# E-J408/admm-net

Measured on AMD Instinct MI355X. Metric: signals/sec (K-layer ADMM-Net forward), higher is better.
Workload: dtype f32; 1 GPU; cfg3: ADMMNet K=16 grid 16x16 (D=256, n=257) batch 65536/GPU + spectrum on 1024 atoms; batch_per_gpu=65536, global_batch=65536, K=16, D=256, n=257, natoms=1024, batch_mean_scope=global, chunk=8192, weights=torch.manual_seed(0) default init, glayer=matrix function, checked per matrix; eigensolver on the rejected matrices

## Files before the change

__graft_entry__.py:

```python
import os
import subprocess
import sys

ROOT = os.path.dirname(os.path.abspath(__file__))
if ROOT not in sys.path:
    sys.path.insert(0, ROOT)


def build() -> None:
    from admm_net_amd import build as b
    lib = b.build_extension()
    assert os.path.exists(lib)
    for name in ("eigh_model", "dc_model", "arrow_model"):
        so = os.path.join(ROOT, "tests", "host_model", "lib%s.so" % name)
        subprocess.check_call(["g++", "-O2", "-shared", "-fPIC", "-I", os.path.join(ROOT, "admm_net_amd", "csrc"),
                               os.path.join(ROOT, "tests", "host_model", name + ".cpp"), "-o", so])
    import admm_net_amd
    from admm_net_amd import _lib
    _lib.load()


def smoke() -> None:
    import numpy as np
    import torch
    import admm_net_amd as A
    from admm_net_amd import synth
    from oracle import admm_net_ref as R
    assert torch.cuda.is_available(), "smoke() needs the GPU"
    dev = torch.device("cuda:0")
    Nb, Nd, K, B = 4, 4, 3, 5
    sd = R.make_weights(Nb, Nd, K, seed=1, head=True, perturb=0.3)
    m = A.ADMMNet(M=Nb, N=Nd, num_layers=K).eval()
    m.load_state_dict(sd)
    y, b, s, _ = synth.make_batch(B, Nb, Nd, seed=2)
    ty, tb, ts = torch.from_numpy(y), torch.from_numpy(b), torch.from_numpy(s)
    tau, f, conf, phi = m(ty.to(dev), tb.to(dev), ts.to(dev))
    torch.cuda.synchronize()
    ref = R.forward(sd, ty, tb, ts, Nb, Nd, K, head=True)
    err = float(np.abs(phi.cpu().numpy() - ref[3].numpy()).max() / np.abs(ref[3].numpy()).max())
    herr = max(float((a.cpu() - r).abs().max()) for a, r in zip((tau, f, conf), ref[:3]))
    assert err < 1e-4 and herr < 5e-5, (err, herr)
    st = m.last_status
    print(f"smoke ok: phi rel err {err:.2e}, head abs err {herr:.2e}; G-layer routes {st}")


if __name__ == "__main__":
    build()
    if "--smoke" in sys.argv:
        smoke()
```

admm_net_amd/csrc/arrow.hip:

```cpp
#include <cstdio>
#include <cstdlib>

#include "common.h"

#include "arrow_core.h"
#include "rebuild_lds.h"

namespace admmnet {

constexpr int AR_THREADS = 256;

struct ArShared {
    int k, nrot, conf;
    int mx[2];
    float znorm;
};

__host__ __device__ inline size_t ar_np(int D) { return (size_t)((D + 1 + 3) & ~3); }
__host__ __device__ inline size_t ar_lds_bytes(const BrGeom &g) {
    const size_t NP = ar_np(g.D);
    return sizeof(float) * (g.vt_floats() + g.small_floats() + 12 * NP) + sizeof(int) * 5 * NP + sizeof(DcRot) * NP;
}

template <bool BIG>
__global__ __launch_bounds__(AR_THREADS, 1) void arrow_rebuild_kernel(
    int D, const float *__restrict__ lw, const float2 *__restrict__ phi, const float *__restrict__ h,
    float2 *__restrict__ G, float *__restrict__ rn, float *__restrict__ w_out, int32_t *__restrict__ status,
    unsigned long long *__restrict__ ptime, int lower_only, float *VTg, float *__restrict__ w0g) {
    extern __shared__ __attribute__((aligned(16))) char smem[];
    __shared__ ArShared sh;
    long long t_prev = ptime ? clock64() : 0;
    auto mark = [&](int id) {
        if (ptime && threadIdx.x == 0) {
            const long long t_now = clock64();
            atomicAdd(&ptime[id], (unsigned long long)(t_now - t_prev));
            t_prev = t_now;
        }
    };
    const BrGeom g(D);
    const int n = g.n;
    const int Dp = BIG ? D : g.Dp, VP = BIG ? 2 * D : g.VP;
    const int NP = (int)ar_np(D);
    const int tid = threadIdx.x;
    const int64_t b = blockIdx.x;
    const float alpha = lw[S_CORNER_G];
    float *VTl = BIG ? VTg + b * ((int64_t)n * 2 * D) : reinterpret_cast<float *>(smem);
    float *fs = reinterpret_cast<float *>(smem) + (BIG ? 0 : g.vt_floats());
    float *w0f = fs + ((n + 4) & ~3);
    float *z0s = w0f + ((n + 4) & ~3);
    float *rowb = z0s + ((n + 4) & ~3);
    float *redb = rowb + 2 * Dp;
    float *hraw = redb + 8;
    float *zraw = hraw + NP;
    float *phr = zraw + NP;
    float *phim = phr + NP;
    float *ds = phim + NP;
    float *zs = ds + NP;
    float *dl = zs + NP;
    float *zl = dl + NP;
    float *tau = zl + NP;
    float *zh = tau + NP;
    float *vals = zh + NP;
    float *x0 = vals + NP;
    float *lamd = zs;
    int *perm = reinterpret_cast<int *>(x0 + NP);
    int *src = perm + NP;
    int *org = src + NP;
    int *rnk = org + NP;
    int *kidx = rnk + NP;
    DcRot *rot = reinterpret_cast<DcRot *>(kidx + NP);

    if (tid == 0) {
        sh.mx[0] = __float_as_int(fabsf(alpha));
        sh.mx[1] = 0;
    }
    int bad = 0;
    for (int i = tid; i < D; i += AR_THREADS) {
        const float2 z = phi[b * D + i];
        const float a = sqrtf(z.x * z.x + z.y * z.y);
        const float ia = a > 0.f ? 1.0f / a : 0.f;
        hraw[i] = h[b * D + i];
        bad |= !(isfinite(a) && isfinite(hraw[i]));
        zraw[i] = a;
        phr[i] = a > 0.f ? z.x * ia : 1.f;
        phim[i] = a > 0.f ? z.y * ia : 0.f;
    }
    if (__syncthreads_or(bad)) {
        if (tid == 0 && status) atomicAdd(status, 1);
        return;
    }
    for (int i = tid; i < D; i += AR_THREADS) {
        const float v = hraw[i];
        int r = 0;
#pragma unroll 8
        for (int q = 0; q < D; ++q) {
            const float u = hraw[q];
            r += (u < v) || (u == v && q < i);
        }
        perm[r] = i;
        ds[r] = v;
        zs[r] = zraw[i];
        atomicMax(&sh.mx[0], __float_as_int(fabsf(v)));
        atomicMax(&sh.mx[1], __float_as_int(zraw[i]));
    }
    __syncthreads();
    {
        const float dmax = __int_as_float(sh.mx[0]), zmax = __int_as_float(sh.mx[1]);
        int trig = 0;
        for (int p = tid; p < D; p += AR_THREADS) trig |= deflate_triggers(p, 1.0f, dmax, zmax, ds, zs) ? 1 : 0;
        if (__syncthreads_or(trig)) {
            const float tol = 8.0f * kEps32 * fmaxf(dmax, zmax);
            float *dde = reinterpret_cast<float *>(kidx);
            defl_par_flags(tid, AR_THREADS, D, 1.0f, tol, ds, zs, org, rnk, tau, zh);
            if (tid == 0) sh.conf = 0;
            __syncthreads();
            defl_par_walk(tid, AR_THREADS, D, tol, ds, zs, org, rnk, tau, zh, vals, x0, dde, &sh.conf);
            __syncthreads();
            if (sh.conf) {
                if (tid == 0) {
                    int k = 0, nr = 0;
                    deflate_scan_tol(D, 1.0f, dmax, zmax, ds, zs, dl, zl, src, rot, k, nr);
                    sh.k = k;
                    sh.nrot = nr;
                }
            } else {
                defl_par_emit(tid, AR_THREADS, D, ds, org, rnk, tau, zh, vals, x0, dde, dl, zl, src, rot, &sh.k, &sh.nrot);
            }
        } else {
            for (int p = tid; p < D; p += AR_THREADS) {
                dl[p] = ds[p];
                zl[p] = zs[p];
                src[p] = p;
            }
            if (tid == 0) {
                sh.k = D;
                sh.nrot = 0;
            }
        }
    }
    __syncthreads();
    mark(0);
    const int k = sh.k, nrot = sh.nrot;
    for (int p = k + tid; p < D; p += AR_THREADS) vals[p + 1] = dl[p];
    for (int p = tid; p < D; p += AR_THREADS) kidx[src[p]] = (p < k) ? p : -(p + 1) - 1;
    if (tid < 64) {
        float s = 0.f;
        for (int i = tid; i < k; i += 64) s = fmaf(zl[i], zl[i], s);
        s = wave_sum(s);
        if (tid == 0) sh.znorm = sqrtf(s);
    }
    __syncthreads();
    if (k == 0) {
        if (tid == 0) vals[0] = alpha;
    } else {
        const float znorm = sh.znorm;
        auto put = [&](int jr, int o, float t) {
            org[jr] = o;
            tau[jr] = t;
            lamd[jr] = dl[o];
            vals[jr] = dl[o] + t;
        };
        const int first = (k + 1 <= AR_THREADS / 2 + 1) ? min(k + 1, AR_THREADS / 2) : min(k + 1, AR_THREADS);
        if (first <= AR_THREADS / 2) {
            const int jr = tid >> 1, sub = tid & 1;
            if (jr < first) {
                int o;
                float t;
                arrow_root(k, jr, alpha, znorm, dl, zl, o, t, nullptr, sub, 2, [](float x) {
                    return x + __builtin_bit_cast(float, __builtin_amdgcn_update_dpp(0, __builtin_bit_cast(int, x), 0xB1,
                                                                                       0xF, 0xF, false));
                });
                if (sub == 0) put(jr, o, t);
            }
        } else if (tid < first) {
            int o;
            float t;
            arrow_root(k, tid, alpha, znorm, dl, zl, o, t);
            put(tid, o, t);
        }
        if (tid < 64) {
            for (int jr = first; jr <= k; ++jr) {
                int o;
                float t;
                arrow_root(k, jr, alpha, znorm, dl, zl, o, t, nullptr, tid, 64, [](float x) { return wave_sum(x); });
                if (tid == 0) put(jr, o, t);
            }
        }
    }
    __syncthreads();
    for (int p = tid; p < n; p += AR_THREADS) bad |= !isfinite(vals[p]);
    mark(1);
    {
        const int G = (2 * k <= AR_THREADS) ? 2 : 1;
        const int sub = (G == 2) ? (tid & 1) : 0;
        auto redm = [G](float x) {
            const float y = __builtin_bit_cast(
                float, __builtin_amdgcn_update_dpp(0, __builtin_bit_cast(int, x), 0xB1, 0xF, 0xF, false));
            return G == 2 ? x * y : x;
        };
        for (int i = (G == 2) ? (tid >> 1) : tid; i < k; i += AR_THREADS / G) {
            const float v = arrow_zhat(k, i, dl, lamd, tau, sub, G, redm);
            if (sub == 0) zh[i] = v;
        }
    }
    for (int s = tid; s < n; s += AR_THREADS) {
        const float v = vals[s];
        int r = 0;
#pragma unroll 8
        for (int q = 0; q < n; ++q) {
            const float u = vals[q];
            r += (u < v) || (u == v && q < s);
        }
        rnk[s] = r;
    }
    __syncthreads();
    {
        const LayerLayout L{D};
        const float thr = lw[S_THR];
        const float *vn = lw + L.off_vn();
        for (int s = tid; s < n; s += AR_THREADS) {
            float xa = 0.f;
            if (s <= k) {
                float nrm = 1.f;
                if (k > 0) {
                    const float dorg = lamd[s], ts = tau[s];
#pragma unroll 4
                    for (int i = 0; i < k; ++i) {
                        const float v = fdiv_fast(zh[i], (dorg - dl[i]) + ts);
                        nrm = fmaf(v, v, nrm);
                    }
                }
                xa = 1.0f / sqrtf(nrm);
            }
            x0[s] = xa;
            const int c = rnk[s];
            const float lam = vals[s];
            const float f = br_eig_map(lam, thr, vn);
            fs[c] = f;
            w0f[c] = xa * f;
            z0s[c] = xa;
            if (w_out) w_out[b * n + c] = lam;
            if (BIG) w0g[b * n + c] = xa;
        }
        if (tid == 0) {
            fs[n] = 0.f;
            w0f[n] = 0.f;
            z0s[n] = 0.f;
        }
    }
    __syncthreads();
    mark(2);
    int *ipos = reinterpret_cast<int *>(hraw);
    for (int p = tid; p < D; p += AR_THREADS) ipos[perm[p]] = p;
    __syncthreads();
    const int nparts = (AR_THREADS / Dp > 0) ? AR_THREADS / Dp : 1;
    const int sper = (n + nparts - 1) / nparts;
    for (int it = tid; it < Dp * nparts; it += AR_THREADS) {
        const int i = it % Dp, part = it / Dp;
        const int s0 = part * sper, s1 = min(n, s0 + sper);
        float *colr = VTl + i, *coli = VTl + Dp + i;
        if (i >= D) {
            for (int c = s0; c < s1; ++c) {
                colr[c * VP] = 0.f;
                coli[c * VP] = 0.f;
            }
            continue;
        }
        const int kd = kidx[ipos[i]];
        if (kd >= 0) {
            const float zi = zh[kd], di = dl[kd];
#pragma unroll 4
            for (int s = s0; s < min(s1, k + 1); ++s) {
                const float v = fdiv_fast(zi, (lamd[s] - di) + tau[s]) * x0[s];
                colr[rnk[s] * VP] = v;
            }
            for (int s = max(s0, k + 1); s < s1; ++s) colr[rnk[s] * VP] = 0.f;
        } else {
            const int slot = -kd - 1;
#pragma unroll 4
            for (int s = s0; s < s1; ++s) colr[rnk[s] * VP] = (s == slot) ? 1.f : 0.f;
        }
    }
    __syncthreads();
    for (int c = tid; c < n; c += AR_THREADS) {
        float *row = VTl + c * VP;
        for (int r = nrot - 1; r >= 0; --r) {
            const DcRot rr = rot[r];
            const int ia = perm[rr.pa], ib = perm[rr.pb];
            const float a = row[ia], bb = row[ib];
            row[ia] = rr.c * a - rr.s * bb;
            row[ib] = rr.s * a + rr.c * bb;
        }
    }
    __syncthreads();
    for (int it = tid; it < Dp * nparts; it += AR_THREADS) {
        const int i = it % Dp, part = it / Dp;
        if (i >= D) continue;
        float *colr = VTl + i, *coli = VTl + Dp + i;
        const float pr = phr[i], pi = phim[i];
#pragma unroll 8
        for (int c = part * sper; c < min(n, (part + 1) * sper); ++c) {
            const float x = colr[c * VP];
            colr[c * VP] = x * pr;
            coli[c * VP] = x * pi;
        }
    }
    __syncthreads();
    mark(3);
    if (__syncthreads_or(bad) && tid == 0 && status) atomicAdd(status, 1);
    if constexpr (BIG) return;
    else rebuild_from_lds(g, b, lw, VTl, fs, w0f, z0s, rowb, redb, phi, h, G, rn, [&](int id) { mark(id); }, lower_only);
}

bool arrow_rebuild_supported(int D) { return D >= 1 && D <= 256; }

int launch_arrow_rebuild(int D, int64_t nb, const float *lw, const float2 *phi, const float *h, float2 *G, float *rn,
                         float *w_out, int32_t *status, const Ws &ws, hipStream_t st, bool lower_only) {
    if (nb <= 0) return ADMMNET_OK;
    if (!arrow_rebuild_supported(D)) {
        set_error("arrow_rebuild: D=%d unsupported", D);
        return ADMMNET_E_ARG;
    }
    const BrGeom g(D);
    if (D > 128) {
        {
            ProfScope _prof(KC_REBUILD, st);
            const size_t lds = ar_lds_bytes(g) - sizeof(float) * g.vt_floats();
            ADMM_HIP(hipFuncSetAttribute(reinterpret_cast<const void *>(arrow_rebuild_kernel<true>),
                                         hipFuncAttributeMaxDynamicSharedMemorySize, (int)lds));
            hipLaunchKernelGGL(arrow_rebuild_kernel<true>, dim3((unsigned)nb), dim3(AR_THREADS), lds, st, D, lw, phi, h,
                               G, rn, ws.w, status, (unsigned long long *)nullptr, lower_only ? 1 : 0, ws.VT, ws.w0);
            ADMM_HIP(hipGetLastError());
        }
        return launch_rebuild(D, nb, lw, phi, h, G, rn, w_out, ws, st, lower_only, D);
    }
    ProfScope _prof(KC_REBUILD, st);
    const size_t lds = ar_lds_bytes(g);
    ADMM_HIP(hipFuncSetAttribute(reinterpret_cast<const void *>(arrow_rebuild_kernel<false>),
                                 hipFuncAttributeMaxDynamicSharedMemorySize, (int)lds));
    static const bool timing = getenv("ADMMNET_AR_TIMING") != nullptr;
    unsigned long long *ptime = nullptr;
    if (timing) {
        ADMM_HIP(hipMalloc(&ptime, 16 * sizeof(unsigned long long)));
        ADMM_HIP(hipMemsetAsync(ptime, 0, 16 * sizeof(unsigned long long), st));
    }
    hipLaunchKernelGGL(arrow_rebuild_kernel<false>, dim3((unsigned)nb), dim3(AR_THREADS), lds, st, D, lw, phi, h, G, rn,
                       w_out, status, ptime, lower_only ? 1 : 0, (float *)nullptr, (float *)nullptr);
    ADMM_HIP(hipGetLastError());
    if (timing) {
        unsigned long long hb[16];
        ADMM_HIP(hipMemcpyAsync(hb, ptime, sizeof(hb), hipMemcpyDeviceToHost, st));
        ADMM_HIP(hipStreamSynchronize(st));
        ADMM_HIP(hipFree(ptime));
        static const char *nm[6] = {"sort+deflate", "roots", "zhat+rank+norm", "vectors", "G tiles", "arrow+norm"};
        fprintf(stderr, "[arrow_rebuild timing] D=%d nb=%lld  mean cycles per workgroup:\n", D, (long long)nb);
        for (int i = 0; i < 6; ++i) fprintf(stderr, "   %-14s %10.0f\n", nm[i], (double)hb[i] / (double)nb);
    }
    return ADMMNET_OK;
}

}
```

admm_net_amd/csrc/arrow_core.h:

```cpp
#pragma once
#include "dc_core.h"

namespace admmnet {

struct ArrowEval {
    float w, dpsi, dphi, err;
};

struct ArrowNoReduce {
    HD float operator()(float x) const { return x; }
};

template <class DA, class ZA, class Red = ArrowNoReduce>
HD ArrowEval arrow_eval(int k, int jsplit, float c0, float dorg, float t, DA d, ZA z, int sub = 0, int G = 1,
                        Red red = Red()) {
    float sum = 0.f, asum = 0.f, dall = 0.f, dps = 0.f;
#pragma unroll 4
    for (int i = sub; i < k; i += G) {
        const float del = (d(i) - dorg) - t;
        const float r = fdiv_fast(1.0f, del);
        const float zi = z(i);
        const float term = zi * zi * r;
        const float dterm = term * r;
        sum += term;
        asum += fabsf(term);
        dall += dterm;
        dps += (i <= jsplit) ? dterm : 0.f;
    }
    sum = red(sum);
    asum = red(asum);
    dall = red(dall);
    dps = red(dps);
    ArrowEval e;
    e.w = (c0 + t) + sum;
    e.dpsi = dps;
    e.dphi = dall - dps;
    e.err = 8.0f * asum + fabsf(c0) + 2.0f * fabsf(t) + fabsf(t) * dall;
    return e;
}

template <class DA, class ZA, class Red = ArrowNoReduce>
HD void arrow_root_upper(int k, int j, float alpha, float znorm, DA d, ZA z, int &org_out, float &tau_out,
                         int *nit = nullptr, int sub = 0, int G = 1, Red red = Red()) {
    if (nit) *nit = 0;
    const bool top = (j == k);
    int org, plo, phi_;
    float lo, hi, t;
    ArrowEval e;
    if (top) {
        org = k - 1;
        plo = (k >= 2) ? k - 2 : k - 1;
        phi_ = k - 1;
        const float bq = d(k - 1) - alpha;
        const float disc = sqrtf(bq * bq + 4.0f * znorm * znorm);
        hi = (bq > 0.f) ? 2.0f * znorm * znorm / (bq + disc) : 0.5f * (disc - bq);
        lo = 0.f;
        if (k == 1) {
            org_out = org;
            tau_out = hi;
            return;
        }
        hi = hi * (1.0f + 8.0f * kEps32) + 1e-30f;
        t = hi;
        e = arrow_eval(k, plo, d(org) - alpha, d(org), t, d, z, sub, G, red);
        if (e.w <= 0.f) {
            org_out = org;
            tau_out = hi;
            return;
        }
    } else {
        plo = j - 1;
        phi_ = j;
        const float half = 0.5f * (d(j) - d(j - 1));
        e = arrow_eval(k, plo, d(j - 1) - alpha, d(j - 1), half, d, z, sub, G, red);
        if (e.w >= 0.f) {
            org = j - 1;
            lo = 0.f;
            hi = half;
            t = half;
        } else {
            org = j;
            lo = -half;
            hi = 0.f;
            t = -half;
        }
    }
    const float dorg = d(org), c0 = dorg - alpha;
    const float plo_off = d(plo) - dorg, phi_off = d(phi_) - dorg;
    for (int it = 0; it < 60; ++it) {
        if (nit) *nit = it + 1;
        if (fabsf(e.w) <= kEps32 * e.err) break;
        if (e.w < 0.f) lo = t; else hi = t;
        const float d1 = plo_off - t, d2 = phi_off - t;
        const float dw = e.dpsi + e.dphi + 1.0f;
        float c = e.w - d1 * e.dpsi - d2 * e.dphi;
        const float aa = (d1 + d2) * e.w - d1 * d2 * (e.dpsi + e.dphi);
        const float bb = d1 * d2 * e.w;
        float eta;
        if (top) {
            const float zk = z(k - 1), z2 = zk * zk;
            const float psi = e.w - (c0 + t) + fdiv_fast(z2, t);
            const float B = 1.0f + e.dpsi, A = c0 + psi - e.dpsi * t;
            const float disc = sqrtf(A * A + 4.0f * B * z2);
            const float tq = (A > 0.f) ? fdiv_fast(2.0f * z2, A + disc) : fdiv_fast(disc - A, 2.0f * B);
            eta = tq - t;
            (void)c; (void)aa; (void)bb;
        } else {
            if (c == 0.f) {
                eta = (aa != 0.f) ? fdiv_fast(bb, aa) : 0.f;
            } else {
                const float disc = sqrtf(fabsf(aa * aa - 4.0f * bb * c));
                eta = (aa <= 0.f) ? fdiv_fast(aa - disc, 2.0f * c) : fdiv_fast(2.0f * bb, aa + disc);
            }
        }
        if (!(e.w * eta < 0.f)) eta = -fdiv_fast(e.w, dw);
        float tn = t + eta;
        if (!(tn > lo && tn < hi)) tn = 0.5f * (lo + hi);
        if (tn == t || tn == lo || tn == hi) break;
        t = tn;
        e = arrow_eval(k, plo, c0, dorg, t, d, z, sub, G, red);
    }
    if (t == 0.f) t = (lo == 0.f) ? 0.5f * hi : 0.5f * lo;
    if (t == 0.f) t = (lo == 0.f) ? 1e-30f : -1e-30f;
    org_out = org;
    tau_out = t;
}

template <class FA, class Red = ArrowNoReduce>
HD void arrow_root(int k, int j, float alpha, float znorm, FA d, FA z, int &org_out, float &tau_out,
                   int *nit = nullptr, int sub = 0, int G = 1, Red red = Red()) {
    const bool refl = (j == 0);
    const float sg = refl ? -1.0f : 1.0f;
    const int km1 = k - 1;
    int orgr;
    float taur;
    arrow_root_upper(k, refl ? k : j, sg * alpha, znorm, [&](int i) { return sg * d[refl ? km1 - i : i]; },
                     [&](int i) { return z[refl ? km1 - i : i]; }, orgr, taur, nit, sub, G, red);
    org_out = refl ? km1 - orgr : orgr;
    tau_out = sg * taur;
}

template <class FA>
HD float arrow_delta(FA d, FA lamd, FA tau, int i, int j) {
    return (d[i] - lamd[j]) - tau[j];
}

template <class FA, class Red = ArrowNoReduce>
HD float arrow_zhat(int k, int i, FA d, FA lamd, FA tau, int sub = 0, int G = 1, Red red = Red()) {
    const float di = d[i];
    float w = (sub == 0) ? ((di - lamd[i]) - tau[i]) * -((di - lamd[i + 1]) - tau[i + 1])
                         : 1.0f;
#pragma unroll 4
    for (int j = sub; j < k; j += G) {
        const int jr = (j < i) ? j : j + 1;
        const float q = fdiv_fast((di - lamd[jr]) - tau[jr], di - d[j]);
        w *= (j == i) ? 1.0f : q;
    }
    return sqrtf(fabsf(red(w)));
}

}
```

Measured before the change: 87740 signals/s.

## Fuse arrow eigenvector generation and G rebuild into one MFMA kernel for large D

For D>128 the arrow rebuild now runs a fused path by default. Instead of writing the full eigenvector matrix VT to global scratch and running a separate rebuild pass, it generates eigenvector rows in 16-row LDS slabs (double-buffered), undoes the deflation rotations, and accumulates X·diag(f)·X^T with fp32 MFMA 32x32x2 directly. The phase, the arrow row and the residual norm are applied in the epilogue. This removes the global VT round trip and the separate G build, and allows two workgroups per CU, at the cost of register pressure from nine 16-wide accumulators and added complexity in the rotation replay.

After: 92470 signals/s, median of 6. +5.4%, better.

```diff
diff --git a/__graft_entry__.py b/__graft_entry__.py
--- a/__graft_entry__.py
+++ b/__graft_entry__.py
@@ -11,7 +11,7 @@
     from admm_net_amd import build as b
     lib = b.build_extension()
     assert os.path.exists(lib)
-    for name in ("eigh_model", "dc_model", "arrow_model"):
+    for name in ("eigh_model", "dc_model", "arrow_model", "arrow_fused_model"):
         so = os.path.join(ROOT, "tests", "host_model", "lib%s.so" % name)
         subprocess.check_call(["g++", "-O2", "-shared", "-fPIC", "-I", os.path.join(ROOT, "admm_net_amd", "csrc"),
                                os.path.join(ROOT, "tests", "host_model", name + ".cpp"), "-o", so])
diff --git a/admm_net_amd/csrc/arrow.hip b/admm_net_amd/csrc/arrow.hip
--- a/admm_net_amd/csrc/arrow.hip
+++ b/admm_net_amd/csrc/arrow.hip
@@ -9,6 +9,10 @@
 namespace admmnet {
 
 constexpr int AR_THREADS = 256;
+enum ArMode { AR_LDS = 0, AR_GLOBAL = 1, AR_FUSED = 2 };
+constexpr int AF_KS = 16;
+constexpr int AF_W = kMaxD;
+static_assert(AR_THREADS == AF_W, "the fused tail gives every thread one column of X");
 
 struct ArShared {
     int k, nrot, conf;
@@ -22,11 +26,186 @@
     return sizeof(float) * (g.vt_floats() + g.small_floats() + 12 * NP) + sizeof(int) * 5 * NP + sizeof(DcRot) * NP;
 }
 
-template <bool BIG>
-__global__ __launch_bounds__(AR_THREADS, 1) void arrow_rebuild_kernel(
+using f32x16 = __attribute__((ext_vector_type(16))) float;
+
+template <class Mark>
+__device__ __forceinline__ void arrow_fused_tail(int D, int nrot, int64_t b, const float *__restrict__ lw, float *slab,
+                                                 const float *fs, const float *w0f, const float *z0s, const float *lamc,
+                                                 const float *tauc, const float *phr, const float *phim, const float *zh,
+                                                 const float *dl, const int *kidx, int *ipos, const int *perm,
+                                                 const int *rnk, const DcRot *rot, float *redb,
+                                                 const float2 *__restrict__ phi, const float *__restrict__ h,
+                                                 float2 *__restrict__ G, float *__restrict__ rn, int lower_only, Mark mark) {
+    const int n = D + 1, NT = (D + 31) >> 5;
+    const int tid = threadIdx.x, lane = tid & 63;
+    const int wave = __builtin_amdgcn_readfirstlane(tid >> 6);
+    const int r32 = lane & 31, kh = lane >> 5;
+    const int Ihi = 7 - wave, Ilo = wave;
+    for (int p = tid; p < D; p += AR_THREADS) ipos[perm[p]] = p;
+    __syncthreads();
+    float zi = 0.f, di = 0.f;
+    int cdef = -1;
+    bool surv = false;
+    if (tid < D) {
+        const int kd = kidx[ipos[tid]];
+        if (kd >= 0) {
+            surv = true;
+            zi = zh[kd];
+            di = dl[kd];
+        } else {
+            cdef = rnk[-kd - 1];
+        }
+    }
+    auto gen = [&](int sl, int buf) {
+        float *dst = slab + buf * (AF_KS * AF_W) + tid;
+        const int c0 = sl * AF_KS;
+#pragma unroll
+        for (int r = 0; r < AF_KS; ++r) {
+            const int c = c0 + r, cc = min(c, n - 1);
+            const float v = surv ? arrow_vec_entry(zi, di, lamc[cc], tauc[cc], z0s[cc]) : (c == cdef ? 1.f : 0.f);
+            dst[r * AF_W] = (c < n) ? v : 0.f;
+        }
+    };
+    auto unrotate = [&](int sl, int buf) {
+        const int r = tid >> 4;
+        if ((tid & 15) == 0 && sl * AF_KS + r < n) {
+            float *row = slab + (buf * AF_KS + r) * AF_W;
+            for (int q = nrot - 1; q >= 0; --q) {
+                const DcRot rr = rot[q];
+                const int ia = perm[rr.pa], ib = perm[rr.pb];
+                const float a = row[ia], bb = row[ib];
+                row[ia] = rr.c * a - rr.s * bb;
+                row[ib] = rr.s * a + rr.c * bb;
+            }
+        }
+    };
+    const bool hi5 = 5 <= Ihi, hi6 = 6 <= Ihi, hi7 = 7 <= Ihi;
+    const int J5 = hi5 ? 5 : 3, J6 = hi6 ? 6 : 2, J7 = hi7 ? 7 : 1;
+    const bool en_hi = Ihi < NT, en_lo = Ilo < NT;
+    const bool en5 = hi5 ? en_hi : en_lo, en6 = hi6 ? en_hi : en_lo, en7 = hi7 ? en_hi : en_lo;
+    f32x16 acc[9];
+#pragma unroll
+    for (int q = 0; q < 9; ++q) acc[q] = f32x16{0};
+    float arow = 0.f;
+    const int nslab = (n + AF_KS - 1) / AF_KS;
+    gen(0, 0);
+    __syncthreads();
+    if (nrot > 0) {
+        unrotate(0, 0);
+        __syncthreads();
+    }
+    mark(3);
+    auto consume = [&](int sl) {
+        const int c0 = sl * AF_KS;
+        const float *sb = slab + (sl & 1) * (AF_KS * AF_W);
+#pragma unroll
+        for (int r = 0; r < AF_KS; ++r) arow = fmaf(w0f[min(c0 + r, n)], sb[r * AF_W + tid], arow);
+        struct Step { float x0, x1, x2, x3, x4, x5, x6, x7, ahi, alo; };
+        auto load = [&](int kk) {
+            const float fc = fs[min(c0 + kk + kh, n)];
+            const float *row = sb + (kk + kh) * AF_W + r32;
+            return Step{row[0], row[32], row[64], row[96], row[128], row[32 * J5], row[32 * J6], row[32 * J7],
+                        row[32 * Ihi] * fc, row[32 * Ilo] * fc};
+        };
+        Step cur = load(0);
+#pragma unroll
+        for (int kk = 0; kk < AF_KS; kk += 2) {
+            Step nxt = cur;
+            if (kk + 2 < AF_KS) nxt = load(kk + 2);
+            __builtin_amdgcn_sched_barrier(0);
+            if (c0 + kk < n) {
+                const float a5 = hi5 ? cur.ahi : cur.alo, a6 = hi6 ? cur.ahi : cur.alo, a7 = hi7 ? cur.ahi : cur.alo;
+                if (en_hi) {
+                    acc[0] = __builtin_amdgcn_mfma_f32_32x32x2f32(cur.ahi, cur.x0, acc[0], 0, 0, 0);
+                    acc[1] = __builtin_amdgcn_mfma_f32_32x32x2f32(cur.ahi, cur.x1, acc[1], 0, 0, 0);
+                    acc[2] = __builtin_amdgcn_mfma_f32_32x32x2f32(cur.ahi, cur.x2, acc[2], 0, 0, 0);
+                    acc[3] = __builtin_amdgcn_mfma_f32_32x32x2f32(cur.ahi, cur.x3, acc[3], 0, 0, 0);
+                    acc[4] = __builtin_amdgcn_mfma_f32_32x32x2f32(cur.ahi, cur.x4, acc[4], 0, 0, 0);
+                }
+                if (en5) acc[5] = __builtin_amdgcn_mfma_f32_32x32x2f32(a5, cur.x5, acc[5], 0, 0, 0);
+                if (en6) acc[6] = __builtin_amdgcn_mfma_f32_32x32x2f32(a6, cur.x6, acc[6], 0, 0, 0);
+                if (en7) acc[7] = __builtin_amdgcn_mfma_f32_32x32x2f32(a7, cur.x7, acc[7], 0, 0, 0);
+                if (en_lo) acc[8] = __builtin_amdgcn_mfma_f32_32x32x2f32(cur.alo, cur.x0, acc[8], 0, 0, 0);
+            }
+            __builtin_amdgcn_sched_barrier(0);
+            cur = nxt;
+        }
+    };
+    for (int sl = 0; sl < nslab; ++sl) {
+        if (sl + 1 < nslab) gen(sl + 1, (sl & 1) ^ 1);
+        consume(sl);
+        __syncthreads();
+        if (nrot > 0 && sl + 1 < nslab) {
+            unrotate(sl + 1, (sl & 1) ^ 1);
+            __syncthreads();
+        }
+    }
+    mark(4);
+    float2 *Gb = G + b * (int64_t)n * n;
+    float acc2 = 0.f;
+#pragma unroll
+    for (int q = 0; q < 9; ++q) {
+        const bool hi = q <= 4 || (q == 5 && hi5) || (q == 6 && hi6) || (q == 7 && hi7);
+        const int I = hi ? Ihi : Ilo, J = hi ? q : 8 - q;
+        if (I < NT) {
+            const int gj = 32 * J + r32;
+            const float prj = phr[min(gj, D - 1)], pij = phim[min(gj, D - 1)];
+#pragma unroll
+            for (int e = 0; e < 16; ++e) {
+                const int gi = 32 * I + (e & 3) + 8 * (e >> 2) + 4 * kh;
+                if (gi >= gj && gi < D) {
+                    const float S = acc[q][e];
+                    if (gi == gj) {
+                        Gb[(int64_t)gi * n + gj] = make_float2(S, 0.f);
+                        const float d = S - h[b * D + gi];
+                        acc2 += d * d;
+                    } else {
+                        float re, im;
+                        arrow_phase_entry(S, phr[gi], phim[gi], prj, pij, re, im);
+                        Gb[(int64_t)gi * n + gj] = make_float2(re, im);
+                        if (!lower_only) Gb[(int64_t)gj * n + gi] = make_float2(re, -im);
+                        acc2 += 2.f * (re * re + im * im);
+                    }
+                }
+            }
+        }
+    }
+    if (tid < D) {
+        const int o = tid;
+        const float gr = arow * phr[o], gim = -(arow * phim[o]);
+        Gb[(int64_t)D * n + o] = make_float2(gr, gim);
+        if (!lower_only) Gb[(int64_t)o * n + D] = make_float2(gr, -gim);
+        const float2 p = phi[b * D + o];
+        const float dr = gr - p.x, dm = gim + p.y;
+        acc2 += 2.f * (dr * dr + dm * dm);
+    }
+    if (wave == 0) {
+        float g00 = 0.f;
+        for (int c = lane; c < n; c += 64) g00 = fmaf(w0f[c], z0s[c], g00);
+        g00 = wave_sum(g00);
+        if (lane == 0) {
+            Gb[(int64_t)D * n + D] = make_float2(g00, 0.f);
+            const float d = g00 - lw[S_CORNER_Z];
+            acc2 += d * d;
+        }
+    }
+    acc2 = wave_sum(acc2);
+    if (lane == 0) redb[wave] = acc2;
+    __syncthreads();
+    if (tid == 0) {
+        float s = 0.f;
+        for (int i = 0; i < AR_THREADS / 64; ++i) s += redb[i];
+        rn[b] = sqrtf(s);
+    }
+    mark(5);
+}
+
+template <int MODE>
+__global__ __launch_bounds__(AR_THREADS, MODE == AR_FUSED ? 2 : 1) void arrow_rebuild_kernel(
     int D, const float *__restrict__ lw, const float2 *__restrict__ phi, const float *__restrict__ h,
     float2 *__restrict__ G, float *__restrict__ rn, float *__restrict__ w_out, int32_t *__restrict__ status,
     unsigned long long *__restrict__ ptime, int lower_only, float *VTg, float *__restrict__ w0g) {
+    constexpr bool BIG = MODE == AR_GLOBAL, FUSED = MODE == AR_FUSED;
     extern __shared__ __attribute__((aligned(16))) char smem[];
     __shared__ ArShared sh;
     long long t_prev = ptime ? clock64() : 0;
@@ -45,7 +224,7 @@
     const int64_t b = blockIdx.x;
     const float alpha = lw[S_CORNER_G];
     float *VTl = BIG ? VTg + b * ((int64_t)n * 2 * D) : reinterpret_cast<float *>(smem);
-    float *fs = reinterpret_cast<float *>(smem) + (BIG ? 0 : g.vt_floats());
+    float *fs = reinterpret_cast<float *>(smem) + (BIG || FUSED ? 0 : g.vt_floats());
     float *w0f = fs + ((n + 4) & ~3);
     float *z0s = w0f + ((n + 4) & ~3);
     float *rowb = z0s + ((n + 4) & ~3);
@@ -69,6 +248,7 @@
     int *rnk = org + NP;
     int *kidx = rnk + NP;
     DcRot *rot = reinterpret_cast<DcRot *>(kidx + NP);
+    float *lamc = ds, *tauc = zl;
 
     if (tid == 0) {
         sh.mx[0] = __float_as_int(fabsf(alpha));
@@ -241,6 +421,11 @@
             z0s[c] = xa;
             if (w_out) w_out[b * n + c] = lam;
             if (BIG) w0g[b * n + c] = xa;
+            if (FUSED) {
+                const bool root = s <= k && k > 0;
+                lamc[c] = root ? lamd[s] : 3.0e38f;
+                tauc[c] = root ? tau[s] : 0.f;
+            }
         }
         if (tid == 0) {
             fs[n] = 0.f;
@@ -250,6 +435,13 @@
     }
     __syncthreads();
     mark(2);
+    if constexpr (FUSED) {
+        if (__syncthreads_or(bad) && tid == 0 && status) atomicAdd(status, 1);
+        arrow_fused_tail(D, nrot, b, lw, reinterpret_cast<float *>(rot + NP), fs, w0f, z0s, lamc, tauc, phr, phim, zh, dl,
+                         kidx, reinterpret_cast<int *>(hraw), perm, rnk, rot, redb, phi, h, G, rn, lower_only,
+                         [&](int id) { mark(id); });
+        return;
+    }
     int *ipos = reinterpret_cast<int *>(hraw);
     for (int p = tid; p < D; p += AR_THREADS) ipos[perm[p]] = p;
     __syncthreads();
@@ -314,6 +506,27 @@
 
 bool arrow_rebuild_supported(int D) { return D >= 1 && D <= 256; }
 
+struct ArTiming {
+    unsigned long long *d = nullptr;
+    int begin(hipStream_t st) {
+        static const bool on = getenv("ADMMNET_AR_TIMING") != nullptr;
+        if (!on) return ADMMNET_OK;
+        ADMM_HIP(hipMalloc(&d, 16 * sizeof(unsigned long long)));
+        ADMM_HIP(hipMemsetAsync(d, 0, 16 * sizeof(unsigned long long), st));
+        return ADMMNET_OK;
+    }
+    int end(hipStream_t st, int D, int64_t nb, const char *const (&nm)[6]) {
+        if (!d) return ADMMNET_OK;
+        unsigned long long hb[16];
+        ADMM_HIP(hipMemcpyAsync(hb, d, sizeof(hb), hipMemcpyDeviceToHost, st));
+        ADMM_HIP(hipStreamSynchronize(st));
+        ADMM_HIP(hipFree(d));
+        fprintf(stderr, "[arrow_rebuild timing] D=%d nb=%lld  mean cycles per workgroup:\n", D, (long long)nb);
+        for (int i = 0; i < 6; ++i) fprintf(stderr, "   %-14s %10.0f\n", nm[i], (double)hb[i] / (double)nb);
+        return ADMMNET_OK;
+    }
+};
+
 int launch_arrow_rebuild(int D, int64_t nb, const float *lw, const float2 *phi, const float *h, float2 *G, float *rn,
                          float *w_out, int32_t *status, const Ws &ws, hipStream_t st, bool lower_only) {
     if (nb <= 0) return ADMMNET_OK;
@@ -322,13 +535,28 @@
         return ADMMNET_E_ARG;
     }
     const BrGeom g(D);
+    int rc;
+    static const bool fused_env = !(getenv("ADMMNET_ARROW_FUSED") && atoi(getenv("ADMMNET_ARROW_FUSED")) == 0);
+    if (D > 128 && fused_env && !ws.skip) {
+        ProfScope _prof(KC_REBUILD, st);
+        const size_t lds = ar_lds_bytes(g) - sizeof(float) * g.vt_floats() + sizeof(float) * 2 * AF_KS * AF_W;
+        ADMM_HIP(hipFuncSetAttribute(reinterpret_cast<const void *>(arrow_rebuild_kernel<AR_FUSED>),
+                                     hipFuncAttributeMaxDynamicSharedMemorySize, (int)lds));
+        ArTiming tm;
+        if ((rc = tm.begin(st))) return rc;
+        hipLaunchKernelGGL(arrow_rebuild_kernel<AR_FUSED>, dim3((unsigned)nb), dim3(AR_THREADS), lds, st, D, lw, phi, h, G,
+                           rn, w_out, status, tm.d, lower_only ? 1 : 0, (float *)nullptr, (float *)nullptr);
+        ADMM_HIP(hipGetLastError());
+        static const char *const nm[6] = {"sort+deflate", "roots", "zhat+rank+norm", "first slab", "slabs + S", "epilogue"};
+        return tm.end(st, D, nb, nm);
+    }
     if (D > 128) {
         {
             ProfScope _prof(KC_REBUILD, st);
             const size_t lds = ar_lds_bytes(g) - sizeof(float) * g.vt_floats();
-            ADMM_HIP(hipFuncSetAttribute(reinterpret_cast<const void *>(arrow_rebuild_kernel<true>),
+            ADMM_HIP(hipFuncSetAttribute(reinterpret_cast<const void *>(arrow_rebuild_kernel<AR_GLOBAL>),
                                          hipFuncAttributeMaxDynamicSharedMemorySize, (int)lds));
-            hipLaunchKernelGGL(arrow_rebuild_kernel<true>, dim3((unsigned)nb), dim3(AR_THREADS), lds, st, D, lw, phi, h,
+            hipLaunchKernelGGL(arrow_rebuild_kernel<AR_GLOBAL>, dim3((unsigned)nb), dim3(AR_THREADS), lds, st, D, lw, phi, h,
                                G, rn, ws.w, status, (unsigned long long *)nullptr, lower_only ? 1 : 0, ws.VT, ws.w0);
             ADMM_HIP(hipGetLastError());
         }
@@ -336,27 +564,15 @@
     }
     ProfScope _prof(KC_REBUILD, st);
     const size_t lds = ar_lds_bytes(g);
-    ADMM_HIP(hipFuncSetAttribute(reinterpret_cast<const void *>(arrow_rebuild_kernel<false>),
+    ADMM_HIP(hipFuncSetAttribute(reinterpret_cast<const void *>(arrow_rebuild_kernel<AR_LDS>),
                                  hipFuncAttributeMaxDynamicSharedMemorySize, (int)lds));
-    static const bool timing = getenv("ADMMNET_AR_TIMING") != nullptr;
-    unsigned long long *ptime = nullptr;
-    if (timing) {
-        ADMM_HIP(hipMalloc(&ptime, 16 * sizeof(unsigned long long)));
-        ADMM_HIP(hipMemsetAsync(ptime, 0, 16 * sizeof(unsigned long long), st));
-    }
-    hipLaunchKernelGGL(arrow_rebuild_kernel<false>, dim3((unsigned)nb), dim3(AR_THREADS), lds, st, D, lw, phi, h, G, rn,
-                       w_out, status, ptime, lower_only ? 1 : 0, (float *)nullptr, (float *)nullptr);
+    ArTiming tm;
+    if ((rc = tm.begin(st))) return rc;
+    hipLaunchKernelGGL(arrow_rebuild_kernel<AR_LDS>, dim3((unsigned)nb), dim3(AR_THREADS), lds, st, D, lw, phi, h, G, rn,
+                       w_out, status, tm.d, lower_only ? 1 : 0, (float *)nullptr, (float *)nullptr);
     ADMM_HIP(hipGetLastError());
-    if (timing) {
-        unsigned long long hb[16];
-        ADMM_HIP(hipMemcpyAsync(hb, ptime, sizeof(hb), hipMemcpyDeviceToHost, st));
-        ADMM_HIP(hipStreamSynchronize(st));
-        ADMM_HIP(hipFree(ptime));
-        static const char *nm[6] = {"sort+deflate", "roots", "zhat+rank+norm", "vectors", "G tiles", "arrow+norm"};
-        fprintf(stderr, "[arrow_rebuild timing] D=%d nb=%lld  mean cycles per workgroup:\n", D, (long long)nb);
-        for (int i = 0; i < 6; ++i) fprintf(stderr, "   %-14s %10.0f\n", nm[i], (double)hb[i] / (double)nb);
-    }
-    return ADMMNET_OK;
+    static const char *const nm[6] = {"sort+deflate", "roots", "zhat+rank+norm", "vectors", "G tiles", "arrow+norm"};
+    return tm.end(st, D, nb, nm);
 }
 
 }
diff --git a/admm_net_amd/csrc/arrow_core.h b/admm_net_amd/csrc/arrow_core.h
--- a/admm_net_amd/csrc/arrow_core.h
+++ b/admm_net_amd/csrc/arrow_core.h
@@ -159,4 +159,14 @@
     return sqrtf(fabsf(red(w)));
 }
 
+HD float arrow_vec_entry(float zi, float di, float lamd, float tau, float x0) {
+    return fdiv_fast(zi, (lamd - di) + tau) * x0;
 }
+
+HD void arrow_phase_entry(float S, float pri, float pii, float prj, float pij, float &re, float &im) {
+    const float cr = pri * prj + pii * pij, ci = pii * prj - pri * pij;
+    re = S * cr;
+    im = S * ci;
+}
+
+}
```
